# MIT-SPARK/Khronos

Hardware: AMD Instinct MI355X
Metric: active-window frames/sec (+ Mvoxel-updates/sec) at 1280x720 RGB-D+labels, 2 cm voxels (higher is better)
Workload: dtype f32

## Files before the change

### include/khronos_amd.h

```cpp
#ifndef KHRONOS_AMD_H_
#define KHRONOS_AMD_H_

#include <stddef.h>
#include <stdint.h>

#ifdef __cplusplus
extern "C" {
#endif

#define KHR_OK 0
#define KHR_EINVAL (-1)
#define KHR_ENOMEM (-2)
#define KHR_EDEVICE (-3)
#define KHR_ENOTFOUND (-4)
#define KHR_ESTATE (-5)

#define KHR_VOX_ACTIVE 1u
#define KHR_VOX_EVER_FREE 2u
#define KHR_VOX_TO_REMOVE 4u
#define KHR_VOX_SEM_VALID 8u
#define KHR_BLK_UPDATED 1u
#define KHR_BLK_MESH_UPDATED 2u
#define KHR_BLK_TRACKING_UPDATED 4u
#define KHR_BLK_HAS_ACTIVE_DATA 8u
// ... 151 lines not shown
size_t khr_motion_bits_bytes(int64_t n_pixels);
int khr_motion_bits(khr_ctx* ctx, int slot, void* bits_device);
int khr_detect_motion_from_bits(khr_ctx* ctx, int slot, const void* bits_device);
int khr_dynamic_pack_bytes(khr_ctx* ctx, int slot, void* dst_device);
int khr_dynamic_unpack_bytes(khr_ctx* ctx, int slot, const void* src_device);
int khr_mirror_dynamic(khr_ctx* ctx, int src_slot, int dst_slot);
int khr_get_dynamic_clusters(khr_ctx* ctx, int slot, khr_cluster* out, int cap);
int khr_configure_object_detector(khr_ctx* ctx, const khr_object_detector_config* cfg);
int khr_detect_objects(khr_ctx* ctx, int slot);
int khr_detect_objects_launch(khr_ctx* ctx, int slot);
int khr_get_semantic_clusters(khr_ctx* ctx, int slot, khr_cluster* out, int cap);
int64_t khr_cluster_voxels(khr_ctx* ctx, int slot, int which, float voxel_size, int32_t* ids_out, int64_t* voxels_out,
                           int64_t cap);
int khr_cluster_voxels_launch(khr_ctx* ctx, int slot, int which, float voxel_size);
int64_t khr_cluster_voxels_fetch(khr_ctx* ctx, int which, int32_t* ids_out, int64_t* voxels_out, int64_t cap);
typedef struct khr_pixel_ref {
  int32_t slot;
  int32_t which;
  int32_t id;
} khr_pixel_ref;
int khr_pixel_iou(khr_ctx* ctx, int slot, const khr_pixel_ref* refs, int n_refs, int max_id, uint32_t* n_points, uint32_t* inter);
int khr_forward_instances(khr_ctx* ctx, int slot, float max_range, const int32_t* background_ids, int n_background, int max_id,
                          khr_cluster* out);
int khr_generate_mesh(khr_ctx* ctx, int only_mesh_updated, int clear_flag);
#define KHR_MESH_HALO_RECORD_BYTES(vps) (4 * (4 + 3 * 6 * (vps) * (vps)))
int khr_mesh_halo_requests(khr_ctx* ctx, void* keys_out, int64_t cap, int only_mesh_updated, int on_device);
int khr_mesh_halo_export(khr_ctx* ctx, const void* requests, int64_t n_requests, void* records, int64_t cap_records,
                         int on_device);
int khr_mesh_halo_import(khr_ctx* ctx, const void* records, int64_t n_records, int on_device);
#define KHR_MESH_HALO_REQ_HEADER_WORDS(world) (8 * (world))
// ... 220 lines not shown
```

### khronos_amd/capi.py

```python
import ctypes as C
import os

import numpy as np

_HERE = os.path.dirname(os.path.abspath(__file__))
LIB_PATH = os.path.join(_HERE, "lib", "libkhronos_amd.so")

KHR_OK, KHR_EINVAL, KHR_ENOMEM, KHR_EDEVICE, KHR_ENOTFOUND, KHR_ESTATE = 0, -1, -2, -3, -4, -5
VOX_ACTIVE, VOX_EVER_FREE, VOX_TO_REMOVE, VOX_SEM_VALID = 1, 2, 4, 8
BLK_UPDATED, BLK_MESH_UPDATED, BLK_TRACKING_UPDATED, BLK_HAS_ACTIVE_DATA = 1, 2, 4, 8


class KhrConfig(C.Structure):
    _fields_ = [
        ("voxel_size", C.c_float), ("voxels_per_side", C.c_int32), ("truncation_distance", C.c_float),
        ("with_semantics", C.c_int32), ("with_tracking", C.c_int32), ("num_labels", C.c_int32),
        ("use_weight_dropoff", C.c_int32), ("weight_dropoff_epsilon", C.c_float),
        ("use_constant_weight", C.c_int32), ("max_weight", C.c_float), ("interpolation_method", C.c_int32),
        ("adaptive_max_range_difference", C.c_float), ("range_mode", C.c_int32), ("semantic_mode", C.c_int32),
        ("label_confidence", C.c_float),
        ("temporal_buffer", C.c_float), ("tsdf_occupancy_threshold", C.c_float),
        ("neighbor_connectivity", C.c_int32), ("temporal_window", C.c_float),
        ("md_neighbor_connectivity", C.c_int32), ("md_min_cluster_size", C.c_int32),
        ("md_max_cluster_size", C.c_int32), ("md_min_separation_distance", C.c_float),
# ... 112 lines not shown
    "khr_download_block", "khr_mesh_num_vertices", "khr_download_mesh", "khr_fetch_mesh", "khr_fetch_mesh_into", "khr_timing_enable", "khr_timing_reset",
    "khr_timing_get", "khr_debug_read", "khr_tick_ingest", "khr_tick_integrate", "khr_tick_live_bound", "khr_tick_seed_counts", "khr_converted_bytes", "khr_export_converted",
    "khr_converted_views", "khr_tick_adopt", "khr_copy_frame_image", "khr_rv_detect_changes", "khr_last_removed", "khr_process_frame", "khr_ingest_ahead", "khr_ingest_ahead_host", "khr_ingest_cancel", "khr_integrate_shared", "khr_integrate_shared_batch", "khr_pixel_iou", "khr_forward_instances", "khr_update_tracking_phase",
    "khr_export_halo", "khr_import_halo", "khr_get_dynamic_clusters", "khr_motion_keys", "khr_motion_bits_bytes", "khr_motion_bits", "khr_detect_motion_from_bits",
    "khr_dynamic_pack_bytes", "khr_dynamic_unpack_bytes",
    "khr_detect_motion_from_keys", "khr_download_updated", "khr_mesh_halo_requests", "khr_mesh_halo_export",
    "khr_mesh_halo_requests_sorted", "khr_mesh_halo_plan", "khr_mesh_halo_answer", "khr_mesh_halo_adopt",
    "khr_mesh_halo_import", "khr_configure_object_detector", "khr_detect_objects", "khr_get_semantic_clusters",
    "khr_cluster_voxels", "khr_download_frame_image", "khr_detect_objects_launch", "khr_pool_exhausted", "khr_map_digest",
    "khr_rv_create", "khr_rv_destroy", "khr_rv_clear", "khr_rv_add_rays", "khr_rv_num_rays", "khr_rv_num_pairs", "khr_rv_check",
    "khr_snapshot_updated", "khr_take_snapshot", "khr_snapshot_num_blocks", "khr_snapshot_download", "khr_snapshot_download_extra", "khr_snapshot_download_begin", "khr_snapshot_download_end", "khr_snapshot_poll", "khr_fetch_mesh_launch", "khr_reserve_mesh_staging", "khr_reserve_snapshots", "khr_mirror_dynamic", "khr_snapshot_release",
    "khr_rv_check_stamps", "khr_get_config", "khr_cluster_voxels_launch", "khr_cluster_voxels_fetch", "khr_reset_map", "khr_depend_on", "khr_retain_slot", "khr_release_slot",
    "khr_map_slice", "khr_slice_voxel_z", "khr_render_view", "khr_query_points",
    "khr_align_linearize", "khr_align_frame", "khr_distance_field",
    "khr_checkpoint_size", "khr_checkpoint_save", "khr_checkpoint_load", "khr_checkpoint_inspect",
    "khr_debug_live_resources",
]

_lib = None


class KhronosAmdError(RuntimeError):
    pass


def load_library():
    global _lib
    if _lib is not None:
        return _lib
    if not os.path.exists(LIB_PATH):
        raise KhronosAmdError(
# ... 39 lines not shown
    lib.khr_rv_num_rays.argtypes = [vp]
    lib.khr_rv_num_rays.restype = C.c_int64
    lib.khr_rv_num_pairs.argtypes = [vp]
    lib.khr_rv_num_pairs.restype = C.c_int64
    lib.khr_rv_check.argtypes = [vp, C.c_int64, vp, vp, vp, vp, vp, C.POINTER(C.c_uint64), C.POINTER(C.c_uint64)]
    lib.khr_rv_check_stamps.argtypes = [vp, vp, vp]
    lib.khr_rv_detect_changes.argtypes = [vp, C.c_float, C.c_int64, i32, C.c_float, C.c_float, vp, i32, vp, vp, vp]
    lib.khr_get_config.argtypes = [vp, vp]
    lib.khr_reset_map.argtypes = [vp, C.c_float, C.c_float]
    lib.khr_depend_on.argtypes = [vp, vp]
    lib.khr_retain_slot.argtypes = [vp, i32]
    lib.khr_release_slot.argtypes = [vp, i32]
    lib.khr_cluster_voxels_launch.argtypes = [vp, i32, i32, C.c_float]
    lib.khr_cluster_voxels_fetch.argtypes = [vp, i32, vp, vp, C.c_int64]
    lib.khr_cluster_voxels_fetch.restype = C.c_int64
    lib.khr_get_semantic_clusters.argtypes = [vp, i32, C.POINTER(KhrCluster), i32]
    lib.khr_cluster_voxels.argtypes = [vp, i32, i32, C.c_float, vp, vp, C.c_int64]
    lib.khr_cluster_voxels.restype = C.c_int64
    lib.khr_generate_mesh.argtypes = [vp, i32, i32]
    lib.khr_reset_inactive.argtypes = [vp, vp, i64, C.POINTER(i64)]
    lib.khr_mark_all_inactive.argtypes = [vp]
    lib.khr_clear_updated.argtypes = [vp]
    lib.khr_allocate_blocks.argtypes = [vp, vp, i64]
    lib.khr_object_prune.argtypes = [vp, C.c_float, C.c_float, C.POINTER(i64)]
    lib.khr_get_stats.argtypes = [vp, C.POINTER(KhrStats)]
    lib.khr_num_blocks.argtypes = [vp]
    lib.khr_num_blocks.restype = i64
    lib.khr_block_indices.argtypes = [vp, vp, i64, i32]
    lib.khr_block_indices.restype = i64
    lib.khr_download_block.argtypes = [vp, C.c_int32, C.c_int32, C.c_int32] + [vp] * 9
# ... 407 lines not shown
                                                     int(max_id), arr))
        out = [dict(id=a.id, num_pixels=a.num_pixels_listed, bbox_min=np.array(a.bbox_min[:]), bbox_max=np.array(a.bbox_max[:]),
                    centroid=np.array(a.centroid[:])) for a in arr if a.num_pixels_listed]
        assert len(out) == n
        return out

    def cluster_voxels(self, slot, which, voxel_size):
        n = self.lib.khr_cluster_voxels(self.h, slot, which, float(voxel_size), None, None, 0)
        self._chk(n)
        ids = np.zeros(max(n, 1), np.int32)
        vox = np.zeros((max(n, 1), 3), np.int64)
        n2 = self.lib.khr_cluster_voxels(self.h, slot, which, float(voxel_size), _ptr(ids), _ptr(vox), n)
        self._chk(n2)
        return ids[:n], vox[:n]

    def generate_mesh(self, only_mesh_updated=True, clear_flag=True):
        self._chk(self.lib.khr_generate_mesh(self.h, int(only_mesh_updated), int(clear_flag)))

    def reset_inactive(self):
        n = C.c_int64(0)
        cap = int(self.cfg.max_blocks)
        out = np.zeros((cap, 3), np.int32)
        self._chk(self.lib.khr_reset_inactive(self.h, _ptr(out), cap, C.byref(n)))
        return out[: n.value].copy()

    def reset_inactive_async(self):
        self._chk(self.lib.khr_reset_inactive(self.h, None, 0, None))

    def mark_all_inactive(self):
        self._chk(self.lib.khr_mark_all_inactive(self.h))
# ... 569 lines not shown
```

### khronos_amd/csrc/khr_kernels_objects.h

```cpp
#pragma once
#include "khr_device.h"

namespace khr {

constexpr int kGvWindow = 32766;
constexpr uint32_t kGvMaxGroup = 32766;
constexpr uint32_t kNodeNone = 0xffffffffu, kNodeOwner = 0x80000000u;

__host__ __device__ inline uint64_t gvKey(uint32_t group, int rx, int ry, int rz) {
  return (static_cast<uint64_t>(group) << 48) | (static_cast<uint64_t>(static_cast<uint32_t>(rx + 32768) & 0xffffu) << 32) |
         (static_cast<uint64_t>(static_cast<uint32_t>(ry + 32768) & 0xffffu) << 16) |
         static_cast<uint64_t>(static_cast<uint32_t>(rz + 32768) & 0xffffu);
}
__host__ __device__ inline uint64_t gvOriginKey(uint32_t group) { return static_cast<uint64_t>(group) << 48; }
__host__ __device__ inline bool gvIsOrigin(uint64_t k) { return (k & 0xffffffffffffull) == 0ull; }
__host__ __device__ inline void gvUnpack(uint64_t k, uint32_t* group, int* rx, int* ry, int* rz) {
  *group = static_cast<uint32_t>(k >> 48);
  *rx = static_cast<int>((k >> 32) & 0xffffu) - 32768;
  *ry = static_cast<int>((k >> 16) & 0xffffu) - 32768;
  *rz = static_cast<int>(k & 0xffffu) - 32768;
}

struct GvTable {
  uint64_t* keys;
// ... 388 lines not shown
        atomicOr(&flags[0], 2u);
      } else {
        float pw[3];
        pixelVertex(f, i, pw);
        has = gvVoxelKey(pw, inv, origin, static_cast<uint32_t>(id), !(f.range[i] > 0.f), &key);
        if (!has) atomicOr(&flags[0], 1u);
      }
    }
  }
  bool claimed;
  const uint32_t h = gvInsertWave(t, has, key, &claimed);
  const uint64_t my_key = key;
  const uint32_t at = waveAggInc(n_list, claimed);
  if (claimed && at < cap) {
    list[at] = my_key;
    slots[at] = h;
  }
}


constexpr int kPixRefs = 32;
struct PixRefs {
  int n;
  int32_t id[kPixRefs];
  int32_t bit[kPixRefs];
};
struct PixCamera {
  double T[12];
  float fx, fy, cx, cy;
  int W, H;
// ... 173 lines not shown
```

### khronos_amd/csrc/khronos_amd.hip

```cpp
#include <hip/hip_runtime.h>
#include <hip/hip_ext.h>
#include <hipcub/hipcub.hpp>

#include <algorithm>
#include <array>
#include <atomic>
#include <chrono>
#include <memory>
#include <mutex>
#include <cmath>
#include <cstdarg>
#include <cstdio>
#include <climits>
#include <cstring>
#include <cstdlib>
#include <functional>
#include <map>
#include <string>
#include <thread>
#include <tuple>
#include <unordered_map>
#include <vector>

#include "../../include/khronos_amd.h"
// ... 69 lines not shown
  bool dyn_clean = false;
  bool dynw_valid = false;
  uint64_t aux_seq = 0;
  std::vector<khr_cluster> sem_clusters;
  std::vector<khr_cluster> clusters;
};

struct TimingRec {
  int which;
  Event a, b;
};

constexpr int kNumTimers = 13;
constexpr uint32_t kObjHead = 512;
constexpr uint32_t kCvHead = 8192;
constexpr uint32_t kCompCap = 1024, kCompHead = 64;

}

struct khr_ctx {
  khr_config cfg{};
  DevParams p{};
  DevMap m{};
  int device = 0;
  Stream stream;
  Stream aux_stream;
  Stream copy_stream;
  Stream snap_stream;
  Stream mc_stream;
  Stream h2d_stream;
  Event ev_aux, ev_aux_done;
  uint64_t aux_seq_issued = 0, aux_seq_done = 0, obj_seq = 0, cv_seq[2] = {0, 0};
  std::vector<DevBuf<uint8_t>> allocs;
  std::vector<FrameSlot> slots;
  int next_slot = 0;
  std::unique_ptr<std::atomic<int>[]> slot_leases;
  uint32_t* d_work = nullptr;
  uint32_t* d_new = nullptr;
  uint32_t* d_ef = nullptr;
  uint32_t* d_trk_proc = nullptr;
  uint32_t* d_tick_work = nullptr;
  uint32_t* d_tick_counts = nullptr;
  uint32_t* d_tick_seeds = nullptr;
  PinnedBuf<uint32_t> h_tick;
  uint32_t tick_ticket = 0;
  std::vector<uint32_t> tick_seed_host;
  int tick_seed_n = 0, tick_seed_collected = 0;
// ... 155 lines not shown
  bool obj_configured = false;
  khr_object_detector_config obj_cfg{};
  std::vector<int32_t> obj_labels;
  DevBuf<int32_t> d_obj_labels;
  uint64_t* d_gv_keys = nullptr;
  uint32_t gv_mask = 0;
  uint32_t *d_gv_parent = nullptr, *d_gv_rootidx = nullptr, *d_gv_node = nullptr;
  uint32_t* d_gv_n = nullptr;
  ObjAcc* d_obj_acc = nullptr;
  int32_t* d_obj_final = nullptr;
  uint64_t* d_cv_list = nullptr;
  uint32_t obj_root_cap = 0;
  uint32_t* d_gv_owners = nullptr;
  uint32_t* d_gv_done = nullptr;
  bool gv_clean = false;
  bool gv_counters_clean[3] = {false, false, false};
  PinnedBuf<uint8_t> h_obj_head;
  Event ev_obj;
  int obj_pending_slot = -1;
  uint32_t* d_cv_n[2] = {nullptr, nullptr};
  uint64_t* d_cv_keys[2] = {nullptr, nullptr};
  PinnedBuf<uint8_t> h_cv[2];
  Event ev_cv[2];
  int cv_pending_slot[2] = {-1, -1};
  uint32_t obj_ticket = 0, cv_ticket[2] = {0, 0};
  int3 cv_origin[2]{};
  MeshBuffers mesh[2]{};
  int mesh_cur = 0;
  uint32_t *d_mesh_count = nullptr, *d_mesh_offset = nullptr;
  uint8_t* d_regen = nullptr;
  uint32_t* d_mesh_old_off = nullptr;
  uint32_t* d_mesh_nwork = nullptr;
  uint64_t mesh_total = 0;
  bool mesh_stale = false;
  std::vector<uint32_t> h_counters;
  khr_stats stats{};
  bool host_index_valid = false;
  std::map<std::array<int32_t, 3>, uint32_t> host_index;
  std::vector<uint32_t> host_flags;
  DevBuf<uint64_t> d_slice_keys;
  DevBuf<uint32_t> d_slice_count;
// ... 732 lines not shown
    return fail(KHR_EINVAL, "bad intrinsics / range");
  HIP_TRY(hipSetDevice(c->device));
  const int slot = acquireSlot(c);
  if (slot < 0) return slot;
  FrameSlot& s = c->slots[slot];
  const hipMemcpyKind kind = on_device ? hipMemcpyDeviceToDevice : hipMemcpyHostToDevice;
  s.valid = false;
  s.sensor = *sensor;
  s.meta = *frame;
  s.meta.depth = nullptr;
  s.meta.color = nullptr;
  s.meta.label = nullptr;
  s.has_color = frame->color != nullptr;
  s.has_label = frame->label != nullptr;
  s.has_obj = false;
  s.objects_done = false;
  s.clusters.clear();
  s.sem_clusters.clear();
  const bool pinned = !on_device && c->host_input_pinned;
  hipStream_t ist = ((on_device || pinned) && c->ingest_stream) ? c->ingest_stream : c->stream;
  ScopedTimer tm(c, ist == c->stream ? 6 : -1);
  const float* depth_src = frame->depth;
  const uint8_t* rgb_src = frame->color;
  const int32_t* label_src = frame->label;
  if (!on_device) {
    hipStream_t cs = c->stream;
    if (pinned) {
      if (!c->h2d_stream) KHR_TRY(createStream(c, c->h2d_stream));
      KHR_TRY((c->h2d_ev_target ? *c->h2d_ev_target : c->ev_h2d).ensure());
      cs = c->h2d_stream;
// ... 35 lines not shown
  return slot;
}

int khr_set_frame_image(khr_ctx* c, int slot, int which, const int32_t* image, int on_device) {
  if (!c || slot < 0 || slot >= static_cast<int>(c->slots.size()) || !c->slots[slot].valid) return fail(KHR_EINVAL, "bad slot");
  FrameSlot& s = c->slots[slot];
  const size_t n = static_cast<size_t>(s.sensor.width) * s.sensor.height;
  int32_t* dst = which == 0 ? s.dyn : s.obj;
  if (image) {
    HIP_TRY(hipMemcpyAsync(dst, image, n * sizeof(int32_t), on_device ? hipMemcpyDeviceToDevice : hipMemcpyHostToDevice, c->stream));
    if (!on_device) HIP_TRY(hipStreamSynchronize(c->stream));
  } else {
    HIP_TRY(hipMemsetAsync(dst, 0, n * sizeof(int32_t), c->stream));
  }
  if (which == 1) s.has_obj = image != nullptr;
  if (which == 0) s.dyn_clean = image == nullptr;
  if (which == 0) s.dynw_valid = false;
  if (which == 1) {
    const int rca = auxAfterMain(c);
    if (rca) return rca;
  }
  return KHR_OK;
}

int khr_download_frame(khr_ctx* c, int slot, float* range, float* vertex_map, int32_t* dynamic_image) {
  if (!c || slot < 0 || slot >= static_cast<int>(c->slots.size()) || !c->slots[slot].valid) return fail(KHR_EINVAL, "bad slot");
  FrameSlot& s = c->slots[slot];
  const size_t n = static_cast<size_t>(s.sensor.width) * s.sensor.height;
  if (range) HIP_TRY(hipMemcpyAsync(range, s.vRange(), n * sizeof(float), hipMemcpyDeviceToHost, c->stream));
  if (dynamic_image) HIP_TRY(hipMemcpyAsync(dynamic_image, s.dyn, n * sizeof(int32_t), hipMemcpyDeviceToHost, c->stream));
// ... 579 lines not shown
  for (int base = 0; base < n_frames; base += kMaxTick) {
    const int nb = std::min(kMaxTick, n_frames - base);
    TickIngest t{};
    for (int k = 0; k < nb; ++k) {
      const khr_frame& fr = frames[base + k];
      const int slot = slots_out[base + k];
      FrameSlot& s = c->slots[slot];
      s.sensor = *sensor;
      s.meta = fr;
      s.meta.depth = nullptr;
      s.meta.color = nullptr;
      s.meta.label = nullptr;
      s.has_color = fr.color != nullptr;
      s.has_label = fr.label != nullptr;
      s.has_obj = false;
      s.objects_done = false;
      s.clusters.clear();
      s.sem_clusters.clear();
      s.tw = tw;
      s.th = th;
      s.valid = true;
      s.dyn_clean = true, s.dynw_valid = false;
      t.depth_in[k] = fr.depth; t.rgb_in[k] = fr.color; t.label_in[k] = fr.label;
      t.depth[k] = s.depth; t.range[k] = s.range; t.rgba[k] = s.rgba; t.label[k] = s.label; t.dyn[k] = s.dyn;
      t.tile_max[k] = s.tile_max;
      float R[9], tt[3];
      makePose(fr.world_T_sensor, R, tt, t.Rw[k], t.tw[k]);
      t.min_z_world[k] = static_cast<float>(fr.world_T_sensor[11] + static_cast<double>(c->cfg.md_min_z_coordinate));
    }
    hipLaunchKernelGGL(k_tick_ingest, dim3(tw * th, nb), dim3(256), 0, c->stream, t, tw, sensor->width, sensor->height, sensor->fx,
// ... 86 lines not shown
  if ((rc = acquireTickSlots(c, n_frames, slots_out))) return rc;
  TickSlotsGuard undo{c, slots_out, n_frames};
  for (int base = 0; base < n_frames; base += kMaxTick) {
    const int nb = std::min(kMaxTick, n_frames - base);
    TickAdopt t{};
    for (int k = 0; k < nb; ++k) {
      const khr_converted_frame& fr = frames[base + k];
      FrameSlot& s = c->slots[slots_out[base + k]];
      s.sensor = *sensor;
      s.meta = khr_frame{};
      s.meta.timestamp_ns = fr.timestamp_ns;
      std::memcpy(s.meta.world_T_sensor, fr.world_T_sensor, sizeof(s.meta.world_T_sensor));
      s.has_color = fr.rgba != nullptr;
      s.has_label = fr.label != nullptr;
      s.has_obj = false;
      s.objects_done = false;
      s.clusters.clear();
      s.sem_clusters.clear();
      s.tw = tw;
      s.th = th;
      s.valid = true;
      s.dyn_clean = true, s.dynw_valid = false;
      s.x_range = fr.range;
      s.x_depth = fr.depth ? fr.depth : fr.range;
      s.x_rgba = fr.rgba;
      s.x_label = fr.label;
      s.x_tile_max = fr.tile_max;
      t.range[k] = fr.range;
      t.depth[k] = fr.depth;
      t.dyn[k] = s.dyn;
// ... 943 lines not shown
  c->obj_root_cap = 1u << 16;
  int rc = KHR_OK;
  KHR_CHAIN(devAlloc(c, &c->d_gv_keys, ts, false));
  KHR_CHAIN(devAlloc(c, &c->d_gv_parent, ts, false));
  KHR_CHAIN(devAlloc(c, &c->d_gv_rootidx, ts, false));
  KHR_CHAIN(devAlloc(c, &c->d_gv_node, npx, false));
  KHR_CHAIN(devAlloc(c, &c->d_gv_owners, npx, false));
  KHR_CHAIN(devAlloc(c, &c->d_gv_done, 4));
  {
    uint8_t* head = nullptr;
    KHR_CHAIN(devAlloc(c, &head, 16 + sizeof(ObjAcc) * c->obj_root_cap));
    c->d_gv_n = reinterpret_cast<uint32_t*>(head);
    c->d_obj_acc = head ? reinterpret_cast<ObjAcc*>(head + 16) : nullptr;
  }
  KHR_CHAIN(devAlloc(c, &c->d_obj_final, c->obj_root_cap, false));
  for (int w = 0; w < 2; ++w) {
    uint8_t* head = nullptr;
    KHR_CHAIN(devAlloc(c, &head, 16 + sizeof(uint64_t) * npx));
    c->d_cv_n[w] = reinterpret_cast<uint32_t*>(head);
    c->d_cv_keys[w] = head ? reinterpret_cast<uint64_t*>(head + 16) : nullptr;
    KHR_CHAIN(c->h_cv[w].alloc(16 + sizeof(uint64_t) * npx));
    KHR_CHAIN(c->ev_cv[w].ensure());
  }
  KHR_CHAIN(c->h_obj_head.alloc(16 + sizeof(ObjAcc) * c->obj_root_cap));
  KHR_CHAIN(c->ev_obj.ensure());
  if (rc == KHR_OK && hipStreamSynchronize(c->stream) != hipSuccess) rc = KHR_EDEVICE;
  return rc;
}

static int3 windowOrigin(const DevFrame& f, float inv) {
  return make_int3(static_cast<int>(std::floor(f.tw[0] * inv)), static_cast<int>(std::floor(f.tw[1] * inv)),
// ... 21 lines not shown
    HIP_TRY(hipStreamSynchronize(c->stream));
  }
  c->obj_configured = true;
  return KHR_OK;
}

static int objectsLaunch(khr_ctx* c, int slot) {
  FrameSlot& s = c->slots[slot];
  const int n = s.sensor.width * s.sensor.height;
  const khr_object_detector_config& oc = c->obj_cfg;
  s.sem_clusters.clear();
  s.objects_done = false;
  s.has_obj = true;
  s.aux_seq = c->obj_seq = ++c->aux_seq_issued;
  c->obj_pending_slot = -1;
  const int n_labels = static_cast<int>(c->obj_labels.size());
  if (!s.has_label || n_labels == 0) {
    HIP_TRY(hipMemsetAsync(s.obj, 0, sizeof(int32_t) * n, c->aux_stream));
    s.objects_done = true;
    return KHR_OK;
  }
  const DevFrame f = makeDevFrame(c, s);
  GvTable t{c->d_gv_keys, c->gv_mask};
  const uint32_t tsize = c->gv_mask + 1;
  if (oc.use_3d) {
    const float inv = 1.f / oc.grid_size;
    if (!c->gv_clean) hipLaunchKernelGGL(k_gv_clear, dim3(gridFor(tsize / 2)), dim3(256), 0, c->aux_stream, c->d_gv_keys, tsize, c->d_gv_n);
    else if (!c->gv_counters_clean[0]) HIP_TRY(hipMemsetAsync(c->d_gv_n, 0, sizeof(uint32_t) * 4, c->aux_stream));
    c->gv_clean = false;
    c->gv_counters_clean[0] = false;
// ... 5 lines not shown
                       c->d_gv_rootidx, c->d_gv_n, c->obj_root_cap, c->d_obj_acc, c->d_gv_keys);
  } else {
    HIP_TRY(hipMemsetAsync(c->d_gv_n, 0, sizeof(uint32_t) * 4, c->aux_stream));
    hipLaunchKernelGGL(k_obj_init2d, dim3(gridFor(n)), dim3(256), 0, c->aux_stream, f, c->d_obj_labels, n_labels, c->d_gv_parent, c->d_gv_node);
    hipLaunchKernelGGL(k_obj_union2d, dim3(gridFor(n)), dim3(256), 0, c->aux_stream, f, c->d_gv_node, c->d_gv_parent,
                       oc.use_full_connectivity ? 1 : 0);
    hipLaunchKernelGGL(k_obj_roots, dim3(gridFor(n)), dim3(256), 0, c->aux_stream, c->d_gv_node, n, c->d_gv_parent, c->d_gv_rootidx, c->d_gv_n,
                       c->obj_root_cap, c->d_obj_acc, nullptr, s.vLabel(), c->d_obj_labels, n_labels);
  }
  const int obj_tiles = ((s.sensor.width + kObjTile - 1) / kObjTile) * ((s.sensor.height + kObjTile - 1) / kObjTile);
  hipLaunchKernelGGL(k_obj_paint, dim3(obj_tiles), dim3(1024), 0, c->aux_stream, f, c->d_gv_node, c->d_gv_parent, c->d_gv_rootidx,
                     c->obj_root_cap, s.obj, c->d_obj_acc);
  HIP_TRY(hipGetLastError());
  if (++c->obj_ticket == 0) ++c->obj_ticket;
  if (oc.use_3d) {
    hipLaunchKernelGGL(k_gv_release_publish, dim3(256), dim3(256), 0, c->aux_stream, c->d_gv_owners, c->d_gv_n + 2, c->d_gv_keys, c->d_gv_done,
                       c->d_gv_n, reinterpret_cast<uint32_t*>(c->h_obj_head.dev()), static_cast<uint32_t>(sizeof(ObjAcc) / 4), kObjHead,
                       c->h_pinned.dev() + 4, c->obj_ticket, c->d_gv_n);
    c->gv_clean = true;
  } else {
    hipLaunchKernelGGL(k_publish, dim3(1), dim3(1024), 0, c->aux_stream, c->d_gv_n, reinterpret_cast<uint32_t*>(c->h_obj_head.dev()),
                       static_cast<uint32_t>(sizeof(ObjAcc) / 4), kObjHead, c->h_pinned.dev() + 4, c->obj_ticket, c->d_gv_n);
  }
  HIP_TRY(hipGetLastError());
  c->gv_counters_clean[0] = oc.use_3d != 0;
  c->obj_pending_slot = slot;
  return KHR_OK;
}

static int objectsFinish(khr_ctx* c, int slot) {
  FrameSlot& s = c->slots[slot];
  if (s.objects_done) return static_cast<int>(s.sem_clusters.size());
  if (c->obj_pending_slot != slot) return fail(KHR_ESTATE, "object detection was not launched for this slot");
  c->obj_pending_slot = -1;
  const int n = s.sensor.width * s.sensor.height;
  const khr_object_detector_config& oc = c->obj_cfg;
  {
    const int rcw = waitTicket(c, 4, c->obj_ticket, "the object detector's cluster records", c->aux_stream);
    if (rcw) return rcw;
    c->aux_seq_done = std::max(c->aux_seq_done, c->obj_seq);
  }
// ... 31 lines not shown
    khr_cluster k{};
    k.id = id;
    k.num_pixels_listed = a.n_pixels;
    k.num_pixels_painted = a.n_pixels;
    for (int d = 0; d < 3; ++d) {
      k.bbox_min[d] = orderedToFloat(a.bmin[d]);
      k.bbox_max[d] = orderedToFloat(a.bmax[d]);
      k.centroid[d] = a.sum[d] / static_cast<float>(a.n_pixels);
    }
    k.semantic_id = c->obj_labels[a.group];
    s.sem_clusters.push_back(k);
  }
  if (R <= static_cast<uint32_t>(kRemapTab)) {
    RemapTab tab{};
    std::memcpy(tab.v, fin.data(), sizeof(int32_t) * R);
    hipLaunchKernelGGL(k_obj_remap_tab, dim3(gridFor(n)), dim3(256), 0, c->aux_stream, s.obj, n, tab);
  } else {
    std::memcpy(c->h_obj_head, fin.data(), sizeof(int32_t) * R);
    HIP_TRY(hipMemcpyAsync(c->d_obj_final, c->h_obj_head, sizeof(int32_t) * R, hipMemcpyHostToDevice, c->aux_stream));
    hipLaunchKernelGGL(k_obj_remap, dim3(gridFor(n)), dim3(256), 0, c->aux_stream, s.obj, n, c->d_obj_final);
  }
  HIP_TRY(hipGetLastError());
  return static_cast<int>(s.sem_clusters.size());
}

int khr_detect_objects(khr_ctx* c, int slot) {
  if (!c || slot < 0 || slot >= static_cast<int>(c->slots.size()) || !c->slots[slot].valid) return fail(KHR_EINVAL, "bad slot");
  if (!c->obj_configured) return fail(KHR_ESTATE, "khr_configure_object_detector has not been called");
  HIP_TRY(hipSetDevice(c->device));
  FrameSlot& s = c->slots[slot];
  if (s.objects_done) return static_cast<int>(s.sem_clusters.size());
// ... 14 lines not shown
  int rc = auxAfterMain(c);
  if (!rc) rc = objectsLaunch(c, slot);
  return rc;
}

int khr_get_semantic_clusters(khr_ctx* c, int slot, khr_cluster* out, int cap) {
  if (!c || cap < 0 || (!out && cap > 0)) return fail(KHR_EINVAL, "bad argument");
  if (slot < 0 || slot >= static_cast<int>(c->slots.size()) || !c->slots[slot].valid) return fail(KHR_EINVAL, "bad slot");
  const FrameSlot& s = c->slots[slot];
  if (!s.objects_done) return fail(KHR_ESTATE, "khr_detect_objects has not run for this frame");
  const int n = static_cast<int>(s.sem_clusters.size());
  for (int i = 0; i < n && i < cap; ++i) out[i] = s.sem_clusters[i];
  return n;
}

int khr_cluster_voxels_launch(khr_ctx* c, int slot, int which, float voxel_size) {
  if (!c || slot < 0 || slot >= static_cast<int>(c->slots.size()) || !c->slots[slot].valid) return fail(KHR_EINVAL, "bad slot");
  if (!(voxel_size > 0.f) || (which != 0 && which != 1)) return fail(KHR_EINVAL, "bad argument");
  HIP_TRY(hipSetDevice(c->device));
  int rc = ensureGv(c);
  if (rc) return rc;
  FrameSlot& s = c->slots[slot];
  c->cv_pending_slot[which] = slot;
  uint32_t* hc = reinterpret_cast<uint32_t*>(c->h_cv[which].get());
  if (which == 1 && !s.has_obj) {
    hc[0] = hc[1] = 0;
    c->cv_ticket[which] = c->h_pinned[5 + which];
    return KHR_OK;
  }
  const int n = s.sensor.width * s.sensor.height;
  const DevFrame f = makeDevFrame(c, s);
  const float inv = 1.f / voxel_size;
  if (which == 0) {
    rc = auxAfterMain(c);
    if (rc) return rc;
  }
  s.aux_seq = c->cv_seq[which] = ++c->aux_seq_issued;
  c->cv_origin[which] = windowOrigin(f, inv);
  GvTable t{c->d_gv_keys, c->gv_mask};
  const uint32_t tsize = c->gv_mask + 1;
  if (!c->gv_clean) hipLaunchKernelGGL(k_gv_clear, dim3(gridFor(tsize / 2)), dim3(256), 0, c->aux_stream, c->d_gv_keys, tsize, c->d_cv_n[which]);
  else if (!c->gv_counters_clean[1 + which]) HIP_TRY(hipMemsetAsync(c->d_cv_n[which], 0, sizeof(uint32_t) * 4, c->aux_stream));
  c->gv_clean = false;
  c->gv_counters_clean[1 + which] = false;
  hipLaunchKernelGGL(k_cluster_voxels, dim3(gridFor(n)), dim3(256), 0, c->aux_stream, f, which == 0 ? s.dyn : s.obj, inv, c->cv_origin[which], t,
                     c->d_cv_keys[which], c->d_cv_n[which], static_cast<uint32_t>(c->cfg.max_frame_pixels), c->d_cv_n[which] + 1,
                     c->d_gv_owners);
  c->gv_clean = true;
  HIP_TRY(hipGetLastError());
  if (++c->cv_ticket[which] == 0) ++c->cv_ticket[which];
  hipLaunchKernelGGL(k_gv_release_publish, dim3(256), dim3(256), 0, c->aux_stream, c->d_gv_owners, c->d_cv_n[which], c->d_gv_keys, c->d_gv_done,
                     c->d_cv_n[which], reinterpret_cast<uint32_t*>(c->h_cv[which].dev()), 2u,
                     static_cast<uint32_t>(std::min<size_t>(kCvHead, c->cfg.max_frame_pixels)), c->h_pinned.dev() + 5 + which, c->cv_ticket[which],
                     c->d_cv_n[which]);
  HIP_TRY(hipGetLastError());
  c->gv_counters_clean[1 + which] = true;
  return KHR_OK;
}

int64_t khr_cluster_voxels_fetch(khr_ctx* c, int which, int32_t* ids_out, int64_t* voxels_out, int64_t cap) {
  if (!c || (which != 0 && which != 1) || cap < 0 || (cap > 0 && (!ids_out || !voxels_out))) return fail(KHR_EINVAL, "bad argument");
  if (c->cv_pending_slot[which] < 0) return fail(KHR_ESTATE, "khr_cluster_voxels_launch has not been called");
  {
    const int rcw = waitTicket(c, 5 + which, c->cv_ticket[which], "the cluster voxel sets", c->aux_stream);
    if (!rcw) c->aux_seq_done = std::max(c->aux_seq_done, c->cv_seq[which]);
    if (rcw) return rcw;
  }
  const uint32_t* cnt = reinterpret_cast<const uint32_t*>(c->h_cv[which].get());
  if (cnt[1] & 1u) return fail(KHR_EINVAL, "cluster voxels: a measured point lies more than %d voxels from the sensor", kGvWindow);
  if (cnt[1] & 2u) return fail(KHR_EINVAL, "cluster voxels: cluster id above %u", kGvMaxGroup);
  const uint32_t N = cnt[0];
  if (N == 0) return 0;
  if (N > kCvHead) {
    HIP_TRY(hipMemcpyAsync(c->h_cv[which], c->d_cv_n[which], 16 + sizeof(uint64_t) * N, hipMemcpyDeviceToHost, c->aux_stream));
    HIP_TRY(hipStreamSynchronize(c->aux_stream));
  }
  const uint64_t* keys = reinterpret_cast<const uint64_t*>(c->h_cv[which] + 16);
  const int3 origin = c->cv_origin[which];
  struct E { int32_t id; int64_t v[3]; };
  std::vector<E> e(N);
  for (uint32_t i = 0; i < N; ++i) {
    uint32_t g;
    int x, y, z;
    gvUnpack(keys[i], &g, &x, &y, &z);
    e[i].id = static_cast<int32_t>(g);
    if (gvIsOrigin(keys[i])) {
      e[i].v[0] = e[i].v[1] = e[i].v[2] = 0;
    } else {
      e[i].v[0] = static_cast<int64_t>(x) + origin.x;
      e[i].v[1] = static_cast<int64_t>(y) + origin.y;
      e[i].v[2] = static_cast<int64_t>(z) + origin.z;
    }
  }
// ... 88 lines not shown
  ObjAcc* const d_acc = reinterpret_cast<ObjAcc*>(c->d_inst.get());
  uint32_t* const d_flags = reinterpret_cast<uint32_t*>(c->d_inst + sizeof(ObjAcc) * n_acc);
  int32_t* const d_bg = reinterpret_cast<int32_t*>(c->d_inst + sizeof(ObjAcc) * n_acc + 16);
  if (n_background) HIP_TRY(hipMemcpyAsync(d_bg, background_ids, sizeof(int32_t) * n_background, hipMemcpyHostToDevice, c->stream));
  hipLaunchKernelGGL(k_inst_clear, dim3(gridFor(n_acc)), dim3(256), 0, c->stream, d_acc, static_cast<int>(n_acc), d_flags);
  const DevFrame f = makeDevFrame(c, s);
  const int tiles = ((f.W + kObjTile - 1) / kObjTile) * ((f.H + kObjTile - 1) / kObjTile);
  hipLaunchKernelGGL(k_inst_forward, dim3(tiles), dim3(1024), 0, c->stream, f, s.obj, max_range, d_bg, n_background, max_id, d_acc, d_flags);
  HIP_TRY(hipGetLastError());
  std::vector<ObjAcc> acc(n_acc);
  uint32_t flags = 0;
  HIP_TRY(hipMemcpyAsync(acc.data(), d_acc, sizeof(ObjAcc) * n_acc, hipMemcpyDeviceToHost, c->stream));
  HIP_TRY(hipMemcpyAsync(&flags, d_flags, sizeof(flags), hipMemcpyDeviceToHost, c->stream));
  HIP_TRY(hipStreamSynchronize(c->stream));
  s.has_obj = true;
  s.objects_done = true;
  s.sem_clusters.clear();
  if (flags & 1u) return fail(KHR_EINVAL, "an instance id of the label image is outside 1..%d", max_id);
  int present = 0;
  for (size_t id = 0; id < n_acc; ++id) {
    khr_cluster k{};
    const ObjAcc& a = acc[id];
    k.id = static_cast<int32_t>(id);
    k.num_pixels_listed = a.n_pixels;
    k.num_pixels_painted = a.n_pixels;
    k.semantic_id = static_cast<int32_t>(id);
    if (a.n_pixels) {
      ++present;
      for (int d = 0; d < 3; ++d) {
        k.bbox_min[d] = orderedToFloat(a.bmin[d]);
// ... 2488 lines not shown
```

### khronos_amd/host/active_window.h

```cpp
#pragma once
#include <cstdlib>
#include <atomic>
#include <condition_variable>
#include <deque>
#include <functional>
#include <memory>
#include <mutex>
#include <optional>
#include <string>
#include <thread>
#include <unordered_set>
#include <vector>

#include "hydra_compat.h"
#include "mini_yaml.h"

namespace khronos {

using hydra::BlockIndex;
using hydra::BlockIndices;
using hydra::BoundingBox;
using hydra::fromSeconds;
using hydra::InputData;
using hydra::KhronosObjectAttributes;
// ... 201 lines not shown
  void assignClustersToStaticTrack(const FrameData& data, std::unordered_set<int>& associated_objects);
  void assignStaticTracksToCluster(const FrameData& data, std::unordered_set<int>& associated_objects);
  void updateTrackingDuration();
  Track& addNewTrack(const MeasurementCluster& observation, bool is_dynamic);
  void updateTrack(const MeasurementCluster& observation, Track& track, bool is_observation_dynamic) const;
  void computeCentroid(const MeasurementCluster& cluster, float* centroid) const;
  float computeIoU(const MeasurementCluster& cluster, const Track& track) const;
  static float computeIoUVoxels(const std::vector<GlobalIndex>& cluster_voxels, const std::vector<GlobalIndex>& track_voxels);
  static float computeIoUBoundingBox(const BoundingBox& a, const BoundingBox& b);

 private:
  TimeStamp processing_stamp_ = 0;
  int current_track_id_ = 0;
  mutable std::vector<int32_t> scratch_ids_;
  mutable std::vector<int64_t> scratch_voxels_;
  const FrameData* current_ = nullptr;
  mutable std::vector<std::vector<uint32_t>> pix_inter_;
  mutable std::vector<uint64_t> pix_key_;
  mutable int pix_max_id_ = 0;
  void ensurePixelIntersections(size_t track_index) const;
};

class ExternalTracker : public Tracker {
 public:
  struct Config {
    int verbosity = 0;
    float temporal_window = 3.f;
    int min_num_observations = 20;
    static Config fromYaml(const khronos_amd::YamlNode& node);
  } const config;
// ... 229 lines not shown
```

### khronos_amd/host/object_tracking.cpp

```cpp
#include <algorithm>
#include <cmath>
#include <limits>
#include <stdexcept>

#include "active_window.h"

namespace khronos {

namespace {
void chk(int rc, const char* what) {
  if (rc < 0) throw std::runtime_error(std::string(what) + ": " + khr_last_error());
}

std::vector<int> parseIntList(const std::string& scalar) {
  std::vector<int> out;
  std::string tok;
  auto flush = [&]() {
    if (!tok.empty()) {
      out.push_back(std::stoi(tok));
      tok.clear();
    }
  };
  for (char ch : scalar) {
    if ((ch >= '0' && ch <= '9') || ch == '-') tok.push_back(ch);
// ... 197 lines not shown
  pix_key_.clear();
  pix_max_id_ = 0;
  for (const auto& c : data.semantic_clusters) pix_max_id_ = std::max(pix_max_id_, c.id);
  associateTracks(data);
  current_ = nullptr;
  updateTrackingDuration();
}

void MaxIoUTracker::setupTrackMeasurements(FrameData& data) const {
  launchTrackMeasurements(data);
  finishTrackMeasurements(data);
}

void MaxIoUTracker::launchTrackMeasurements(FrameData& data) const {
  if (config.track_by != Config::TrackBy::kVoxels || !data.input.ctx || data.input.slot < 0) return;
  if (!data.semantic_clusters.empty())
    chk(khr_cluster_voxels_launch(data.input.ctx, data.input.slot, 1, config.voxel_size), "khr_cluster_voxels_launch");
  if (!data.dynamic_clusters.empty())
    chk(khr_cluster_voxels_launch(data.input.ctx, data.input.slot, 0, config.voxel_size), "khr_cluster_voxels_launch");
}

void MaxIoUTracker::finishTrackMeasurements(FrameData& data) const {
  if (config.track_by != Config::TrackBy::kVoxels || !data.input.ctx || data.input.slot < 0) return;
  auto fill = [&](std::vector<MeasurementCluster>& clusters, int which) {
    for (auto& c : clusters) c.voxels.clear();
    if (clusters.empty()) return;
    if (scratch_ids_.empty()) {
      scratch_ids_.resize(1u << 16);
      scratch_voxels_.resize(3u << 16);
    }
// ... 329 lines not shown
```

Measured before the change: 4011.

## Fuse object cluster-voxel hashing into the object remap kernel with double-buffered sets

```diff
diff --git a/include/khronos_amd.h b/include/khronos_amd.h
--- a/include/khronos_amd.h
+++ b/include/khronos_amd.h
@@ -189,6 +189,7 @@
                            int64_t cap);
 int khr_cluster_voxels_launch(khr_ctx* ctx, int slot, int which, float voxel_size);
 int64_t khr_cluster_voxels_fetch(khr_ctx* ctx, int which, int32_t* ids_out, int64_t* voxels_out, int64_t cap);
+int khr_configure_object_voxel_sets(khr_ctx* ctx, float voxel_size);
 typedef struct khr_pixel_ref {
   int32_t slot;
   int32_t which;
diff --git a/khronos_amd/capi.py b/khronos_amd/capi.py
--- a/khronos_amd/capi.py
+++ b/khronos_amd/capi.py
@@ -150,7 +150,7 @@
     "khr_map_slice", "khr_slice_voxel_z", "khr_render_view", "khr_query_points",
     "khr_align_linearize", "khr_align_frame", "khr_distance_field",
     "khr_checkpoint_size", "khr_checkpoint_save", "khr_checkpoint_load", "khr_checkpoint_inspect",
-    "khr_debug_live_resources",
+    "khr_debug_live_resources", "khr_configure_object_voxel_sets",
 ]
 
 _lib = None
@@ -220,6 +220,7 @@
     lib.khr_cluster_voxels_launch.argtypes = [vp, i32, i32, C.c_float]
     lib.khr_cluster_voxels_fetch.argtypes = [vp, i32, vp, vp, C.c_int64]
     lib.khr_cluster_voxels_fetch.restype = C.c_int64
+    lib.khr_configure_object_voxel_sets.argtypes = [vp, C.c_float]
     lib.khr_get_semantic_clusters.argtypes = [vp, i32, C.POINTER(KhrCluster), i32]
     lib.khr_cluster_voxels.argtypes = [vp, i32, i32, C.c_float, vp, vp, C.c_int64]
     lib.khr_cluster_voxels.restype = C.c_int64
@@ -657,6 +658,20 @@
         self._chk(n2)
         return ids[:n], vox[:n]
 
+    def configure_object_voxel_sets(self, voxel_size):
+        self._chk(self.lib.khr_configure_object_voxel_sets(self.h, float(voxel_size)))
+
+    def cluster_voxels_launch(self, slot, which, voxel_size):
+        self._chk(self.lib.khr_cluster_voxels_launch(self.h, slot, which, float(voxel_size)))
+
+    def cluster_voxels_fetch(self, which):
+        n = self.lib.khr_cluster_voxels_fetch(self.h, which, None, None, 0)
+        self._chk(n)
+        ids = np.zeros(max(n, 1), np.int32)
+        vox = np.zeros((max(n, 1), 3), np.int64)
+        self._chk(self.lib.khr_cluster_voxels_fetch(self.h, which, _ptr(ids), _ptr(vox), n))
+        return ids[:n], vox[:n]
+
     def generate_mesh(self, only_mesh_updated=True, clear_flag=True):
         self._chk(self.lib.khr_generate_mesh(self.h, int(only_mesh_updated), int(clear_flag)))
 
diff --git a/khronos_amd/csrc/khr_kernels_objects.h b/khronos_amd/csrc/khr_kernels_objects.h
--- a/khronos_amd/csrc/khr_kernels_objects.h
+++ b/khronos_amd/csrc/khr_kernels_objects.h
@@ -426,6 +426,41 @@
   const uint32_t at = waveAggInc(n_list, claimed);
   if (claimed && at < cap) {
     list[at] = my_key;
+    slots[at] = h;
+  }
+}
+
+__global__ __launch_bounds__(256) void k_obj_remap_cluster_voxels(DevFrame f, int32_t* __restrict__ obj, RemapTab tab, float inv, int3 origin,
+                                                                 GvTable t, uint64_t* __restrict__ list, uint32_t* __restrict__ n_list,
+                                                                 uint32_t cap, uint32_t* __restrict__ flags, uint32_t* __restrict__ slots) {
+  __shared__ int32_t s_tab[kRemapTab];
+  s_tab[threadIdx.x] = tab.v[threadIdx.x];
+  __syncthreads();
+  const int i = blockIdx.x * blockDim.x + threadIdx.x;
+  bool has = false;
+  uint64_t key = 0;
+  if (i < f.W * f.H) {
+    const int32_t prov = obj[i];
+    if (prov) {
+      const int32_t id = s_tab[prov - 1];
+      obj[i] = id;
+      if (id > 0) {
+        if (static_cast<uint32_t>(id) > kGvMaxGroup) {
+          atomicOr(&flags[0], 2u);
+        } else {
+          float pw[3];
+          pixelVertex(f, i, pw);
+          has = gvVoxelKey(pw, inv, origin, static_cast<uint32_t>(id), !(f.range[i] > 0.f), &key);
+          if (!has) atomicOr(&flags[0], 1u);
+        }
+      }
+    }
+  }
+  bool claimed;
+  const uint32_t h = gvInsertWave(t, has, key, &claimed);
+  const uint32_t at = waveAggInc(n_list, claimed);
+  if (claimed && at < cap) {
+    list[at] = key;
     slots[at] = h;
   }
 }
diff --git a/khronos_amd/csrc/khronos_amd.hip b/khronos_amd/csrc/khronos_amd.hip
--- a/khronos_amd/csrc/khronos_amd.hip
+++ b/khronos_amd/csrc/khronos_amd.hip
@@ -107,6 +107,7 @@
 constexpr int kNumTimers = 13;
 constexpr uint32_t kObjHead = 512;
 constexpr uint32_t kCvHead = 8192;
+constexpr int kGvReleaseGrid = 64;
 constexpr uint32_t kCompCap = 1024, kCompHead = 64;
 
 }
@@ -123,7 +124,7 @@
   Stream mc_stream;
   Stream h2d_stream;
   Event ev_aux, ev_aux_done;
-  uint64_t aux_seq_issued = 0, aux_seq_done = 0, obj_seq = 0, cv_seq[2] = {0, 0};
+  uint64_t aux_seq_issued = 0, aux_seq_done = 0, obj_seq = 0, cv_seq[3] = {0, 0, 0};
   std::vector<DevBuf<uint8_t>> allocs;
   std::vector<FrameSlot> slots;
   int next_slot = 0;
@@ -309,17 +310,20 @@
   uint32_t* d_gv_owners = nullptr;
   uint32_t* d_gv_done = nullptr;
   bool gv_clean = false;
-  bool gv_counters_clean[3] = {false, false, false};
+  bool gv_counters_clean[4] = {false, false, false, false};
   PinnedBuf<uint8_t> h_obj_head;
   Event ev_obj;
   int obj_pending_slot = -1;
-  uint32_t* d_cv_n[2] = {nullptr, nullptr};
-  uint64_t* d_cv_keys[2] = {nullptr, nullptr};
-  PinnedBuf<uint8_t> h_cv[2];
-  Event ev_cv[2];
+  uint32_t* d_cv_n[3] = {nullptr, nullptr, nullptr};
+  uint64_t* d_cv_keys[3] = {nullptr, nullptr, nullptr};
+  PinnedBuf<uint8_t> h_cv[3];
+  Event ev_cv[3];
   int cv_pending_slot[2] = {-1, -1};
-  uint32_t obj_ticket = 0, cv_ticket[2] = {0, 0};
-  int3 cv_origin[2]{};
+  uint32_t obj_ticket = 0, cv_ticket[3] = {0, 0, 0};
+  int3 cv_origin[3]{};
+  int cv_set_obj = 1;
+  float obj_cv_size = 0.f;
+  int obj_cv_slot = -1;
   MeshBuffers mesh[2]{};
   int mesh_cur = 0;
   uint32_t *d_mesh_count = nullptr, *d_mesh_offset = nullptr;
@@ -1082,6 +1086,7 @@
   s.has_color = frame->color != nullptr;
   s.has_label = frame->label != nullptr;
   s.has_obj = false;
+  if (c->obj_cv_slot == slot) c->obj_cv_slot = -1;
   s.objects_done = false;
   s.clusters.clear();
   s.sem_clusters.clear();
@@ -1147,6 +1152,7 @@
     HIP_TRY(hipMemsetAsync(dst, 0, n * sizeof(int32_t), c->stream));
   }
   if (which == 1) s.has_obj = image != nullptr;
+  if (which == 1 && c->obj_cv_slot == slot) c->obj_cv_slot = -1;
   if (which == 0) s.dyn_clean = image == nullptr;
   if (which == 0) s.dynw_valid = false;
   if (which == 1) {
@@ -1756,6 +1762,7 @@
       s.has_color = fr.color != nullptr;
       s.has_label = fr.label != nullptr;
       s.has_obj = false;
+      if (c->obj_cv_slot == slot) c->obj_cv_slot = -1;
       s.objects_done = false;
       s.clusters.clear();
       s.sem_clusters.clear();
@@ -1872,6 +1879,7 @@
       s.has_color = fr.rgba != nullptr;
       s.has_label = fr.label != nullptr;
       s.has_obj = false;
+      if (c->obj_cv_slot == slots_out[base + k]) c->obj_cv_slot = -1;
       s.objects_done = false;
       s.clusters.clear();
       s.sem_clusters.clear();
@@ -2845,7 +2853,7 @@
     c->d_obj_acc = head ? reinterpret_cast<ObjAcc*>(head + 16) : nullptr;
   }
   KHR_CHAIN(devAlloc(c, &c->d_obj_final, c->obj_root_cap, false));
-  for (int w = 0; w < 2; ++w) {
+  for (int w = 0; w < 3; ++w) {
     uint8_t* head = nullptr;
     KHR_CHAIN(devAlloc(c, &head, 16 + sizeof(uint64_t) * npx));
     c->d_cv_n[w] = reinterpret_cast<uint32_t*>(head);
@@ -2897,6 +2905,7 @@
   s.has_obj = true;
   s.aux_seq = c->obj_seq = ++c->aux_seq_issued;
   c->obj_pending_slot = -1;
+  if (c->obj_cv_slot == slot) c->obj_cv_slot = -1;
   const int n_labels = static_cast<int>(c->obj_labels.size());
   if (!s.has_label || n_labels == 0) {
     HIP_TRY(hipMemsetAsync(s.obj, 0, sizeof(int32_t) * n, c->aux_stream));
@@ -2932,8 +2941,8 @@
   HIP_TRY(hipGetLastError());
   if (++c->obj_ticket == 0) ++c->obj_ticket;
   if (oc.use_3d) {
-    hipLaunchKernelGGL(k_gv_release_publish, dim3(256), dim3(256), 0, c->aux_stream, c->d_gv_owners, c->d_gv_n + 2, c->d_gv_keys, c->d_gv_done,
-                       c->d_gv_n, reinterpret_cast<uint32_t*>(c->h_obj_head.dev()), static_cast<uint32_t>(sizeof(ObjAcc) / 4), kObjHead,
+    hipLaunchKernelGGL(k_gv_release_publish, dim3(kGvReleaseGrid), dim3(256), 0, c->aux_stream, c->d_gv_owners, c->d_gv_n + 2, c->d_gv_keys,
+                       c->d_gv_done, c->d_gv_n, reinterpret_cast<uint32_t*>(c->h_obj_head.dev()), static_cast<uint32_t>(sizeof(ObjAcc) / 4), kObjHead,
                        c->h_pinned.dev() + 4, c->obj_ticket, c->d_gv_n);
     c->gv_clean = true;
   } else {
@@ -2943,6 +2952,20 @@
   HIP_TRY(hipGetLastError());
   c->gv_counters_clean[0] = oc.use_3d != 0;
   c->obj_pending_slot = slot;
+  return KHR_OK;
+}
+
+static int cvTicketWord(int set) { return set == 2 ? 12 : 5 + set; }
+
+static int cvReleasePublish(khr_ctx* c, int set) {
+  c->gv_clean = true;
+  if (++c->cv_ticket[set] == 0) ++c->cv_ticket[set];
+  hipLaunchKernelGGL(k_gv_release_publish, dim3(kGvReleaseGrid), dim3(256), 0, c->aux_stream, c->d_gv_owners, c->d_cv_n[set], c->d_gv_keys,
+                     c->d_gv_done, c->d_cv_n[set], reinterpret_cast<uint32_t*>(c->h_cv[set].dev()), 2u,
+                     static_cast<uint32_t>(std::min<size_t>(kCvHead, c->cfg.max_frame_pixels)), c->h_pinned.dev() + cvTicketWord(set),
+                     c->cv_ticket[set], c->d_cv_n[set]);
+  HIP_TRY(hipGetLastError());
+  c->gv_counters_clean[1 + set] = true;
   return KHR_OK;
 }
 
@@ -3004,7 +3027,27 @@
   if (R <= static_cast<uint32_t>(kRemapTab)) {
     RemapTab tab{};
     std::memcpy(tab.v, fin.data(), sizeof(int32_t) * R);
-    hipLaunchKernelGGL(k_obj_remap_tab, dim3(gridFor(n)), dim3(256), 0, c->aux_stream, s.obj, n, tab);
+    if (c->obj_cv_size > 0.f) {
+      const int set = 3 - c->cv_set_obj;
+      const DevFrame f = makeDevFrame(c, s);
+      const float inv = 1.f / c->obj_cv_size;
+      s.aux_seq = c->cv_seq[set] = ++c->aux_seq_issued;
+      c->cv_origin[set] = windowOrigin(f, inv);
+      GvTable t{c->d_gv_keys, c->gv_mask};
+      const uint32_t tsize = c->gv_mask + 1;
+      if (!c->gv_clean) hipLaunchKernelGGL(k_gv_clear, dim3(gridFor(tsize / 2)), dim3(256), 0, c->aux_stream, c->d_gv_keys, tsize, c->d_cv_n[set]);
+      else if (!c->gv_counters_clean[1 + set]) HIP_TRY(hipMemsetAsync(c->d_cv_n[set], 0, sizeof(uint32_t) * 4, c->aux_stream));
+      c->gv_clean = false;
+      c->gv_counters_clean[1 + set] = false;
+      hipLaunchKernelGGL(k_obj_remap_cluster_voxels, dim3(gridFor(n)), dim3(256), 0, c->aux_stream, f, s.obj, tab, inv, c->cv_origin[set], t,
+                         c->d_cv_keys[set], c->d_cv_n[set], static_cast<uint32_t>(c->cfg.max_frame_pixels), c->d_cv_n[set] + 1, c->d_gv_owners);
+      HIP_TRY(hipGetLastError());
+      const int rcp = cvReleasePublish(c, set);
+      if (rcp) return rcp;
+      c->obj_cv_slot = slot;
+    } else {
+      hipLaunchKernelGGL(k_obj_remap_tab, dim3(gridFor(n)), dim3(256), 0, c->aux_stream, s.obj, n, tab);
+    }
   } else {
     std::memcpy(c->h_obj_head, fin.data(), sizeof(int32_t) * R);
     HIP_TRY(hipMemcpyAsync(c->d_obj_final, c->h_obj_head, sizeof(int32_t) * R, hipMemcpyHostToDevice, c->aux_stream));
@@ -3049,6 +3092,14 @@
   return n;
 }
 
+int khr_configure_object_voxel_sets(khr_ctx* c, float voxel_size) {
+  if (!c) return fail(KHR_EINVAL, "null ctx");
+  if (!(voxel_size >= 0.f) || !std::isfinite(voxel_size)) return fail(KHR_EINVAL, "voxel_size must be >= 0 (0 = off)");
+  if (voxel_size != c->obj_cv_size) c->obj_cv_slot = -1;
+  c->obj_cv_size = voxel_size;
+  return KHR_OK;
+}
+
 int khr_cluster_voxels_launch(khr_ctx* c, int slot, int which, float voxel_size) {
   if (!c || slot < 0 || slot >= static_cast<int>(c->slots.size()) || !c->slots[slot].valid) return fail(KHR_EINVAL, "bad slot");
   if (!(voxel_size > 0.f) || (which != 0 && which != 1)) return fail(KHR_EINVAL, "bad argument");
@@ -3057,10 +3108,16 @@
   if (rc) return rc;
   FrameSlot& s = c->slots[slot];
   c->cv_pending_slot[which] = slot;
-  uint32_t* hc = reinterpret_cast<uint32_t*>(c->h_cv[which].get());
+  if (which == 1 && c->obj_cv_slot == slot && c->obj_cv_size == voxel_size && s.has_obj) {
+    c->cv_set_obj = 3 - c->cv_set_obj;
+    c->obj_cv_slot = -1;
+    return KHR_OK;
+  }
+  const int set = which == 0 ? 0 : c->cv_set_obj;
+  uint32_t* hc = reinterpret_cast<uint32_t*>(c->h_cv[set].get());
   if (which == 1 && !s.has_obj) {
     hc[0] = hc[1] = 0;
-    c->cv_ticket[which] = c->h_pinned[5 + which];
+    c->cv_ticket[set] = c->h_pinned[cvTicketWord(set)];
     return KHR_OK;
   }
   const int n = s.sensor.width * s.sensor.height;
@@ -3070,48 +3127,41 @@
     rc = auxAfterMain(c);
     if (rc) return rc;
   }
-  s.aux_seq = c->cv_seq[which] = ++c->aux_seq_issued;
-  c->cv_origin[which] = windowOrigin(f, inv);
+  s.aux_seq = c->cv_seq[set] = ++c->aux_seq_issued;
+  c->cv_origin[set] = windowOrigin(f, inv);
   GvTable t{c->d_gv_keys, c->gv_mask};
   const uint32_t tsize = c->gv_mask + 1;
-  if (!c->gv_clean) hipLaunchKernelGGL(k_gv_clear, dim3(gridFor(tsize / 2)), dim3(256), 0, c->aux_stream, c->d_gv_keys, tsize, c->d_cv_n[which]);
-  else if (!c->gv_counters_clean[1 + which]) HIP_TRY(hipMemsetAsync(c->d_cv_n[which], 0, sizeof(uint32_t) * 4, c->aux_stream));
+  if (!c->gv_clean) hipLaunchKernelGGL(k_gv_clear, dim3(gridFor(tsize / 2)), dim3(256), 0, c->aux_stream, c->d_gv_keys, tsize, c->d_cv_n[set]);
+  else if (!c->gv_counters_clean[1 + set]) HIP_TRY(hipMemsetAsync(c->d_cv_n[set], 0, sizeof(uint32_t) * 4, c->aux_stream));
   c->gv_clean = false;
-  c->gv_counters_clean[1 + which] = false;
-  hipLaunchKernelGGL(k_cluster_voxels, dim3(gridFor(n)), dim3(256), 0, c->aux_stream, f, which == 0 ? s.dyn : s.obj, inv, c->cv_origin[which], t,
-                     c->d_cv_keys[which], c->d_cv_n[which], static_cast<uint32_t>(c->cfg.max_frame_pixels), c->d_cv_n[which] + 1,
+  c->gv_counters_clean[1 + set] = false;
+  hipLaunchKernelGGL(k_cluster_voxels, dim3(gridFor(n)), dim3(256), 0, c->aux_stream, f, which == 0 ? s.dyn : s.obj, inv, c->cv_origin[set], t,
+                     c->d_cv_keys[set], c->d_cv_n[set], static_cast<uint32_t>(c->cfg.max_frame_pixels), c->d_cv_n[set] + 1,
                      c->d_gv_owners);
-  c->gv_clean = true;
   HIP_TRY(hipGetLastError());
-  if (++c->cv_ticket[which] == 0) ++c->cv_ticket[which];
-  hipLaunchKernelGGL(k_gv_release_publish, dim3(256), dim3(256), 0, c->aux_stream, c->d_gv_owners, c->d_cv_n[which], c->d_gv_keys, c->d_gv_done,
-                     c->d_cv_n[which], reinterpret_cast<uint32_t*>(c->h_cv[which].dev()), 2u,
-                     static_cast<uint32_t>(std::min<size_t>(kCvHead, c->cfg.max_frame_pixels)), c->h_pinned.dev() + 5 + which, c->cv_ticket[which],
-                     c->d_cv_n[which]);
-  HIP_TRY(hipGetLastError());
-  c->gv_counters_clean[1 + which] = true;
-  return KHR_OK;
+  return cvReleasePublish(c, set);
 }
 
 int64_t khr_cluster_voxels_fetch(khr_ctx* c, int which, int32_t* ids_out, int64_t* voxels_out, int64_t cap) {
   if (!c || (which != 0 && which != 1) || cap < 0 || (cap > 0 && (!ids_out || !voxels_out))) return fail(KHR_EINVAL, "bad argument");
   if (c->cv_pending_slot[which] < 0) return fail(KHR_ESTATE, "khr_cluster_voxels_launch has not been called");
+  const int set = which == 0 ? 0 : c->cv_set_obj;
   {
-    const int rcw = waitTicket(c, 5 + which, c->cv_ticket[which], "the cluster voxel sets", c->aux_stream);
-    if (!rcw) c->aux_seq_done = std::max(c->aux_seq_done, c->cv_seq[which]);
+    const int rcw = waitTicket(c, cvTicketWord(set), c->cv_ticket[set], "the cluster voxel sets", c->aux_stream);
+    if (!rcw) c->aux_seq_done = std::max(c->aux_seq_done, c->cv_seq[set]);
     if (rcw) return rcw;
   }
-  const uint32_t* cnt = reinterpret_cast<const uint32_t*>(c->h_cv[which].get());
+  const uint32_t* cnt = reinterpret_cast<const uint32_t*>(c->h_cv[set].get());
   if (cnt[1] & 1u) return fail(KHR_EINVAL, "cluster voxels: a measured point lies more than %d voxels from the sensor", kGvWindow);
   if (cnt[1] & 2u) return fail(KHR_EINVAL, "cluster voxels: cluster id above %u", kGvMaxGroup);
   const uint32_t N = cnt[0];
   if (N == 0) return 0;
   if (N > kCvHead) {
-    HIP_TRY(hipMemcpyAsync(c->h_cv[which], c->d_cv_n[which], 16 + sizeof(uint64_t) * N, hipMemcpyDeviceToHost, c->aux_stream));
+    HIP_TRY(hipMemcpyAsync(c->h_cv[set], c->d_cv_n[set], 16 + sizeof(uint64_t) * N, hipMemcpyDeviceToHost, c->aux_stream));
     HIP_TRY(hipStreamSynchronize(c->aux_stream));
   }
-  const uint64_t* keys = reinterpret_cast<const uint64_t*>(c->h_cv[which] + 16);
-  const int3 origin = c->cv_origin[which];
+  const uint64_t* keys = reinterpret_cast<const uint64_t*>(c->h_cv[set] + 16);
+  const int3 origin = c->cv_origin[set];
   struct E { int32_t id; int64_t v[3]; };
   std::vector<E> e(N);
   for (uint32_t i = 0; i < N; ++i) {
@@ -3230,6 +3280,7 @@
   HIP_TRY(hipMemcpyAsync(&flags, d_flags, sizeof(flags), hipMemcpyDeviceToHost, c->stream));
   HIP_TRY(hipStreamSynchronize(c->stream));
   s.has_obj = true;
+  if (c->obj_cv_slot == slot) c->obj_cv_slot = -1;
   s.objects_done = true;
   s.sem_clusters.clear();
   if (flags & 1u) return fail(KHR_EINVAL, "an instance id of the label image is outside 1..%d", max_id);
diff --git a/khronos_amd/host/active_window.h b/khronos_amd/host/active_window.h
--- a/khronos_amd/host/active_window.h
+++ b/khronos_amd/host/active_window.h
@@ -239,6 +239,7 @@
   int current_track_id_ = 0;
   mutable std::vector<int32_t> scratch_ids_;
   mutable std::vector<int64_t> scratch_voxels_;
+  mutable khr_ctx* voxel_sets_ctx_ = nullptr;
   const FrameData* current_ = nullptr;
   mutable std::vector<std::vector<uint32_t>> pix_inter_;
   mutable std::vector<uint64_t> pix_key_;
diff --git a/khronos_amd/host/object_tracking.cpp b/khronos_amd/host/object_tracking.cpp
--- a/khronos_amd/host/object_tracking.cpp
+++ b/khronos_amd/host/object_tracking.cpp
@@ -235,6 +235,10 @@
 
 void MaxIoUTracker::launchTrackMeasurements(FrameData& data) const {
   if (config.track_by != Config::TrackBy::kVoxels || !data.input.ctx || data.input.slot < 0) return;
+  if (voxel_sets_ctx_ != data.input.ctx) {
+    chk(khr_configure_object_voxel_sets(data.input.ctx, config.voxel_size), "khr_configure_object_voxel_sets");
+    voxel_sets_ctx_ = data.input.ctx;
+  }
   if (!data.semantic_clusters.empty())
     chk(khr_cluster_voxels_launch(data.input.ctx, data.input.slot, 1, config.voxel_size), "khr_cluster_voxels_launch");
   if (!data.dynamic_clusters.empty())
```

After: 4114, median of 6. +2.6%, better.
